# lightas/CVPR2020_MANet

Measured on AMD Instinct MI355X. Metric: propagated frames/sec at 480p, 5-frame memory, higher is better.
Workload: dtype f32; 1 GPU; BASELINE configs[1]: grid 120x214, C=100, 5-frame fully-labelled bank (M=128400), 2 ids, f32 arithmetic on f32-stored iid embeddings; step = frame prepare + global match + fused normalise/min-merge + local match d=12; bank sorted/packed once per clip, timed; frames_per_gpu=633, clip_frames=633, bank_exchange=none (1 GPU)

## Files before the change

### cvpr2020_manet_amd/csrc/global_match.hip

```cpp
#include "manet_common.h"
#include <type_traits>
#include "local_geom.h"

namespace {

constexpr int QT = 256;
constexpr int QB = 32;
constexpr int BT = 64;
constexpr int META_INTS = 256;
constexpr int META_T = 0;
constexpr int META_SEG = 1;
constexpr int META_CNT = 130;
constexpr int META_KMAX = 200;
constexpr int META_NAN = 66;
int refine_sub(long T_max) { return T_max <= 2500 ? 8 : 16; }
constexpr int REFINE_XCHG_MASK = 3;
constexpr int REFINE_CAP = 128;
constexpr int REFINE_LDS_LIST = 2048;
constexpr int REFINE_DENSE_CAP = 1024;
constexpr unsigned REFINE_DENSE_BIT = 0x80000000u;
constexpr int REFINE_DENSE_MIN = 64;
constexpr int REFINE_DENSE_LANES = 16;
constexpr int REFINE_RZ = 4;
constexpr int ONE_ROUND_OK = 1 << 29;
// ... 670 lines not shown
    return (u & 0x80000000u) ? ~u : (u | 0x80000000u);
}
__device__ __forceinline__ float float_of(unsigned k)
{
    unsigned u = (k & 0x80000000u) ? (k & 0x7fffffffu) : ~k;
    return __uint_as_float(u);
}

__device__ __forceinline__ float min3p(float m, float a, float b)
{
    return __builtin_elementwise_minimum(__builtin_elementwise_minimum(m, a), b);
}

constexpr int FILTER_TAIL_CUTS = 4;
__device__ __forceinline__ bool split_of_block(int b, int nQT, int S, int T, int block_map, int &qt, int &s, int &t0,
                                               int &t1)
{
    const int bm = block_map & 0xff, small_S = (block_map >> 8) & BLOCK_MAP_SMALL_S_MASK;
    bool one_round = T < S && small_S > 0;
    if (!one_round && (block_map & ONE_ROUND_OK) && small_S > 0 && small_S < S) {
        const float rounds = (float)nQT * (float)S / 512.0f;
        const float whole = floorf(rounds), frac = rounds - whole;
        const float last = frac <= 0.0f ? 0.0f : (frac <= 0.5f ? 0.5f : 1.0f);
        const float cost_host = (whole + last) * ((float)T / (float)S + 0.6f);
        const float cost_one = ceilf((float)T / (float)small_S) + 0.6f;
        one_round = cost_one < 0.97f * cost_host;
    }
    if (one_round) {
        const int S2 = small_S < T ? small_S : T;
        qt = b % nQT;
        s = b / nQT;
        if (s >= S2) return false;
        t0 = (int)((long)s * T / S2);
        t1 = (int)((long)(s + 1) * T / S2);
        return t0 < t1;
    }
    if (bm == 0 || bm == 3) {
        const int xcd = b & 7;
        const int idx = b >> 3;
        qt = idx % nQT;
        s = xcd + 8 * (idx / nQT);
        if (bm == 3 && (S & 7) == 0) s = xcd * (S >> 3) + idx / nQT;
    } else if (bm >= 4 && bm <= 7 && (S & 7) == 0) {
        const int PB = bm - 2, S8 = S >> 3;
        const int xcd = b & 7, idx = b >> 3;
        const int g = idx / (nQT * PB), r = idx - g * (nQT * PB);
        const int pbg = (S8 - g * PB) < PB ? (S8 - g * PB) : PB;
        if (pbg <= 0) return false;
        qt = r / pbg;
        s = xcd + 8 * (g * PB + (r - qt * pbg));
        if (qt >= nQT) return false;
    } else if (bm == 1) {
        qt = b % nQT;
        s = b / nQT;
    } else {
        s = b % S;
        qt = b / S;
    }
    t0 = (int)((long)s * T / S);
    t1 = (int)((long)(s + 1) * T / S);
    return t0 < t1;
}

__device__ __forceinline__ bool tapered_split_of_block(int b, int nQT, int S, int T, int &qt, int &s, int &t0, int &t1)
{
    const int xcd = b & 7, idx = b >> 3, S8 = S >> 3;
    const int full = nQT * (S8 - 1);
    int cut = 0, cuts = 1;
    if (idx < full) {
        qt = idx % nQT;
        s = xcd * S8 + idx / nQT;
    } else {
        const int r = idx - full;
        cut = r / nQT;
        cuts = FILTER_TAIL_CUTS;
        if (cut >= FILTER_TAIL_CUTS) return false;
        qt = r - cut * nQT;
        s = xcd * S8 + S8 - 1;
    }
    const int a = (int)((long)s * T / S), e = (int)((long)(s + 1) * T / S);
    t0 = a + (int)((long)cut * (e - a) / cuts);
    t1 = a + (int)((long)(cut + 1) * (e - a) / cuts);
    return t0 < t1;
}


template <int K>
__device__ __forceinline__ void topk_insert(float (&m)[K], float d)
{
#pragma unroll
    for (int j = 0; j < K; ++j) {
        float lo = fminf(m[j], d);
        d = fmaxf(m[j], d);
        m[j] = lo;
    }
}

template <int KS, int KNN, bool ARG = false, bool NTH = false>
__global__ __launch_bounds__(256, ((KS == 64 && (KNN > 1 || ARG)) || NTH) ? 1 : 2) void global_match_f32_kernel(const char *__restrict__ qpack,
                                                                  const char *__restrict__ bpack,
                                                                  const int *__restrict__ meta,
                                                                  int n_ids, int nQT, int S,
                                                                  long N_pad,
                                                                  unsigned *__restrict__ keys,
                                                                  float *__restrict__ topk, int block_map)
{
    static_assert(!ARG || KNN == 1, "arg-min tracking is the k = 1 path");
    static_assert(!NTH || ARG, "the bounded form is a variant of the arg-min form");
    unsigned long long *keys64 = (unsigned long long *)topk;
    const unsigned long long *bound64 = (const unsigned long long *)keys;
    constexpr int NG = (KS + 3) / 4;
    constexpr size_t TILE_BYTES = bank_tile_bytes(NG);
    constexpr size_t QBLK_BYTES = query_block_bytes(NG);
    extern __shared__ __attribute__((aligned(16))) char smem[];

    const int tid = threadIdx.x;
    const int lane = tid & 63;
    const int wave = __builtin_amdgcn_readfirstlane(tid >> 6);
    const int l31 = lane & 31;
    const int h = lane >> 5;

    int qt, s, t0, t1;
    const int T = meta[META_T];
    if (!split_of_block(blockIdx.x, nQT, S, T, block_map, qt, s, t0, t1)) return;

    constexpr int NV = (int)(TILE_BYTES / 16);
    constexpr int NLD = (NV + 255) / 256;
    u32x4 R[NLD];
#define MANET_GLOAD(R_, t_)                                                                \
    {                                                                                      \
        const u32x4 *g_ = (const u32x4 *)(bpack + (size_t)(t_) * TILE_BYTES);              \
        _Pragma("unroll") for (int i_ = 0; i_ < NLD; ++i_)                                 \
        {                                                                                  \
            const int idx_ = i_ * NTHR + tid;                                              \
            R_[i_] = g_[idx_ < NV ? idx_ : NV - 1];   \
        }                                                                                  \
    }
#define MANET_LSTORE(R_, slot_)                                                            \
    {                                                                                      \
        u32x4 *l_ = (u32x4 *)(smem + (size_t)(slot_) * TILE_BYTES);                        \
        _Pragma("unroll") for (int i_ = 0; i_ < NLD; ++i_)                                 \
            if (i_ * NTHR + tid < NV) l_[i_ * NTHR + tid] = R_[i_];                        \
    }
    constexpr int NTHR = 256;
    MANET_GLOAD(R, t0);

    f32x4 q0[NG], q1[NG];
    float xs0, xs1;
    {
        const char *qb0 = qpack + (size_t)(qt * (QT / QB) + wave * 2) * QBLK_BYTES;
        const char *qb1 = qb0 + QBLK_BYTES;
#pragma unroll
        for (int g = 0; g < NG; ++g) {
            q0[g] = *(const f32x4 *)(qb0 + ((size_t)(g * 2 + h) * QB + l31) * 16);
            q1[g] = *(const f32x4 *)(qb1 + ((size_t)(g * 2 + h) * QB + l31) * 16);
        }
        xs0 = *(const float *)(qb0 + (size_t)NG * 2 * QB * 16 + l31 * 4);
        xs1 = *(const float *)(qb1 + (size_t)NG * 2 * QB * 16 + l31 * 4);
    }
    const long qbase = (long)qt * QT + wave * 64 + l31;

    int o = 0;
    while (meta[META_SEG + o + 1] <= t0) ++o;
    int seg_end = meta[META_SEG + o + 1];
    float m0[KNN], m1[KNN];
    int a0 = -1, a1 = -1;
    unsigned long long B0 = ~0ull, B1 = ~0ull, lo0 = 0, lo1 = 0;
    auto reset = [&]() {
#pragma unroll
        for (int j = 0; j < KNN; ++j) m0[j] = m1[j] = (KNN == 1) ? MANET_WRONG_LABEL_PADDING_DISTANCE : INFINITY;
        a0 = a1 = -1;
        B0 = B1 = ~0ull;
    };
    auto load_bounds = [&](int obj) {
        if (NTH) {
            lo0 = bound64[(size_t)obj * N_pad + qbase];
            lo1 = bound64[(size_t)obj * N_pad + qbase + 32];
        }
    };
    reset();
    load_bounds(o);

    auto flush = [&](int obj) {
        if (ARG) {
            unsigned long long k0 = ((unsigned long long)key_of(m0[0]) << 32) | (unsigned)(a0 < 0 ? -1 : a0 + 4 * h);
            unsigned long long k1 = ((unsigned long long)key_of(m1[0]) << 32) | (unsigned)(a1 < 0 ? -1 : a1 + 4 * h);
            if (NTH) {
                k0 = B0;
                k1 = B1;
            }
            const unsigned long long o0 = __shfl_xor(k0, 32), o1 = __shfl_xor(k1, 32);
            k0 = k0 < o0 ? k0 : o0;
            k1 = k1 < o1 ? k1 : o1;
            if (h == 0) {
                atomicMin(keys64 + (size_t)obj * N_pad + qbase, k0);
                atomicMin(keys64 + (size_t)obj * N_pad + qbase + 32, k1);
            }
        } else if (KNN == 1) {
            float a = min3p(m0[0], m0[0], __shfl_xor(m0[0], 32));
            float c = min3p(m1[0], m1[0], __shfl_xor(m1[0], 32));
            if (h == 0) {
                atomicMin(keys + (size_t)obj * N_pad + qbase, key_of(a));
                atomicMin(keys + (size_t)obj * N_pad + qbase + 32, key_of(c));
            }
        } else {
            float o0[KNN], o1[KNN];
#pragma unroll
            for (int j = 0; j < KNN; ++j) {
                o0[j] = __shfl_xor(m0[j], 32);
                o1[j] = __shfl_xor(m1[j], 32);
            }
#pragma unroll
            for (int j = 0; j < KNN; ++j) {
                topk_insert<KNN>(m0, o0[j]);
                topk_insert<KNN>(m1, o1[j]);
            }
            if (h == 0) {
                float *p0 = topk + (((size_t)s * n_ids + obj) * N_pad + qbase) * KNN;
                float *p1 = p0 + (size_t)32 * KNN;
#pragma unroll
                for (int j = 0; j < KNN; ++j) {
                    p0[j] = m0[j];
                    p1[j] = m1[j];
                }
            }
        }
    };

    MANET_LSTORE(R, 0);
    if (t0 + 1 < t1) MANET_GLOAD(R, t0 + 1);
    for (int t = t0; t < t1; ++t) {
        const int buf = (t - t0) & 1;
        __syncthreads();
        if (t + 1 < t1) {
            MANET_LSTORE(R, buf ^ 1);
            if (t + 2 < t1) MANET_GLOAD(R, t + 2);
        }
        if (t >= seg_end) {
            flush(o);
            reset();
            do { ++o; seg_end = meta[META_SEG + o + 1]; } while (t >= seg_end);
            load_bounds(o);
        }
        const char *tb = smem + (size_t)buf * TILE_BYTES;
        const f32x4 *A = (const f32x4 *)tb;
        f32x16 c00 = {0}, c01 = {0}, c10 = {0}, c11 = {0};
#pragma unroll
        for (int g = 0; g < NG; ++g) {
            f32x4 a0 = A[(g * 2 + h) * BT + l31];
            f32x4 a1 = A[(g * 2 + h) * BT + 32 + l31];
#pragma unroll
            for (int j = 0; j < 4; ++j) {
                if (g * 4 + j < KS) {
                    c00 = __builtin_amdgcn_mfma_f32_32x32x2f32(a0[j], q0[g][j], c00, 0, 0, 0);
                    c01 = __builtin_amdgcn_mfma_f32_32x32x2f32(a0[j], q1[g][j], c01, 0, 0, 0);
                    c10 = __builtin_amdgcn_mfma_f32_32x32x2f32(a1[j], q0[g][j], c10, 0, 0, 0);
                    c11 = __builtin_amdgcn_mfma_f32_32x32x2f32(a1[j], q1[g][j], c11, 0, 0, 0);
                }
            }
        }
        const float *ysl = (const float *)(tb + (size_t)NG * 2 * BT * 16);
#pragma unroll
        for (int tq = 0; tq < 4; ++tq) {
            f32x4 y0 = *(const f32x4 *)(ysl + 8 * tq + 4 * h);
            f32x4 y1 = *(const f32x4 *)(ysl + 32 + 8 * tq + 4 * h);
#pragma unroll
            for (int i = 0; i < 4; ++i) {
                const int r = 4 * tq + i;
                const float d00 = fmaf(-2.0f, c00[r], xs0 + y0[i]);
                const float d01 = fmaf(-2.0f, c01[r], xs1 + y0[i]);
                const float d10 = fmaf(-2.0f, c10[r], xs0 + y1[i]);
                const float d11 = fmaf(-2.0f, c11[r], xs1 + y1[i]);
                if (NTH) {
                    const unsigned slot = (unsigned)(t * BT + (r & 3) + 8 * (r >> 2) + 4 * h);
                    const unsigned long long k00 = ((unsigned long long)key_of(d00) << 32) | slot;
                    const unsigned long long k10 = ((unsigned long long)key_of(d10) << 32) | (slot + 32u);
                    const unsigned long long k01 = ((unsigned long long)key_of(d01) << 32) | slot;
                    const unsigned long long k11 = ((unsigned long long)key_of(d11) << 32) | (slot + 32u);
                    if (k00 > lo0 && k00 < B0) B0 = k00;
                    if (k10 > lo0 && k10 < B0) B0 = k10;
                    if (k01 > lo1 && k01 < B1) B1 = k01;
                    if (k11 > lo1 && k11 < B1) B1 = k11;
                } else if (ARG) {
                    const int slot = t * BT + (r & 3) + 8 * (r >> 2);
                    if (d00 < m0[0]) { m0[0] = d00; a0 = slot; }
                    if (d10 < m0[0]) { m0[0] = d10; a0 = slot + 32; }
                    if (d01 < m1[0]) { m1[0] = d01; a1 = slot; }
                    if (d11 < m1[0]) { m1[0] = d11; a1 = slot + 32; }
                } else if (KNN == 1) {
                    m0[0] = min3p(m0[0], d00, d10);
                    m1[0] = min3p(m1[0], d01, d11);
                } else {
                    topk_insert<KNN>(m0, d00);
                    topk_insert<KNN>(m0, d10);
                    topk_insert<KNN>(m1, d01);
                    topk_insert<KNN>(m1, d11);
                }
            }
        }
    }
    flush(o);
}

template <int KS, bool RESCUE = false>
__global__ __launch_bounds__(256, 2) void global_match_f32_pipe_kernel(const char *__restrict__ qpack,
                                                                       const char *__restrict__ bpack,
                                                                       const int *__restrict__ meta, int n_ids,
                                                                       int nQT, int S, long N_pad,
                                                                       unsigned *__restrict__ keys, int block_map,
                                                                       const unsigned *__restrict__ bcnt = nullptr,
                                                                       long bucket_cap = 0)
{
    constexpr int NG = (KS + 3) / 4;
    constexpr size_t TILE_BYTES = bank_tile_bytes(NG);
    constexpr size_t QBLK_BYTES = query_block_bytes(NG);
    constexpr int PIECES = (int)(TILE_BYTES / 1024);
    constexpr int NW = 4;
    extern __shared__ __attribute__((aligned(16))) char smem[];

    const int tid = threadIdx.x;
    const int lane = tid & 63;
    const int wave = __builtin_amdgcn_readfirstlane(tid >> 6);
    const int l31 = lane & 31;
    const int h = lane >> 5;

    int qt, s, t0, t1;
    const int T = meta[META_T];
    if (RESCUE && (block_map & RESCUE_LISTED)) {
        const unsigned *rs = bcnt + 2 * (N_pad >> 5);
        const int nr = (int)rs[0];
        if (nr <= 0) return;
        int Sd = (block_map >> 8) & BLOCK_MAP_RESCUE_MASK;
        if (Sd > 0) {
            const int most_grid = (int)gridDim.x / nr;
            Sd = Sd > most_grid ? most_grid : Sd;
            Sd = Sd < 1 ? 1 : Sd;
        } else {
            const int most_grid = (int)gridDim.x / nr, most_t = T / 8 > 1 ? T / 8 : 1;
            const int most = most_grid < most_t ? most_grid : most_t;
            long best = -1;
            for (int r = 1; r <= 4; ++r) {
                int c = (512 * r) / nr;
                c = c < 1 ? 1 : (c > most ? most : c);
                const long rounds = ((long)nr * c + 511) / 512;
                const long cost = rounds * ((long)(T + c - 1) / c + 6);
                if (best < 0 || cost < best) { best = cost; Sd = c; }
            }
        }
        if ((int)blockIdx.x >= nr * Sd) return;
        s = (int)blockIdx.x / nr;
        qt = (int)rs[1 + ((int)blockIdx.x - s * nr)];
        t0 = (int)((long)s * T / Sd);
        t1 = (int)((long)(s + 1) * T / Sd);
        if (t0 >= t1) return;
    } else {
        if (!split_of_block(blockIdx.x, nQT, S, T, block_map, qt, s, t0, t1)) return;
        if (RESCUE) {
            bool need = false;
            for (int i = 0; i < QT / QB; ++i) {
                const unsigned raw = bcnt[(long)qt * (QT / QB) + i];
                need = need || (raw >> 31) || (long)raw > bucket_cap;
            }
            if (!need) return;
        }
    }

    const unsigned smem_base = __builtin_amdgcn_readfirstlane((unsigned)(size_t)smem);
    auto stage_dma = [&](int t, int slot) __attribute__((always_inline)) {
        const char *g = bpack + (size_t)t * TILE_BYTES + (size_t)lane * 16;
        const unsigned l = smem_base + (unsigned)slot * (unsigned)TILE_BYTES;
#pragma unroll
        for (int i = 0; i < (PIECES + NW - 1) / NW; ++i) {
            const int pc = wave + i * NW;
            if (pc < PIECES) lds_dma16(g + (size_t)pc * 1024, l + (unsigned)pc * 1024u);
        }
    };
    stage_dma(t0, 0);

    f32x4 q0[NG], q1[NG];
    float xs0, xs1;
    {
        const char *qb0 = qpack + (size_t)(qt * (QT / QB) + wave * 2) * QBLK_BYTES;
        const char *qb1 = qb0 + QBLK_BYTES;
#pragma unroll
        for (int g = 0; g < NG; ++g) {
            q0[g] = *(const f32x4 *)(qb0 + ((size_t)(g * 2 + h) * QB + l31) * 16);
            q1[g] = *(const f32x4 *)(qb1 + ((size_t)(g * 2 + h) * QB + l31) * 16);
        }
        xs0 = *(const float *)(qb0 + (size_t)NG * 2 * QB * 16 + l31 * 4);
        xs1 = *(const float *)(qb1 + (size_t)NG * 2 * QB * 16 + l31 * 4);
    }
    const long qbase = (long)qt * QT + wave * 64 + l31;
#pragma unroll
    for (int g = 0; g < NG; ++g) asm volatile("" : "+v"(q0[g]), "+v"(q1[g]));
    asm volatile("" : "+v"(xs0), "+v"(xs1));

    int o = 0;
    while (meta[META_SEG + o + 1] <= t0) ++o;
    int seg_end = meta[META_SEG + o + 1];
    float m0a, m0b, m1a, m1b;
    m0a = m0b = m1a = m1b = MANET_WRONG_LABEL_PADDING_DISTANCE;
    auto flush = [&](int obj) {
        const float v0 = min3p(m0a, m0b, m0b), v1 = min3p(m1a, m1b, m1b);
        const float a = min3p(v0, v0, __shfl_xor(v0, 32));
        const float c = min3p(v1, v1, __shfl_xor(v1, 32));
        if (h == 0) {
            atomicMin(keys + (size_t)obj * N_pad + qbase, key_of(a));
            atomicMin(keys + (size_t)obj * N_pad + qbase + 32, key_of(c));
        }
    };

    f32x16 c00 = {0}, c01 = {0}, c10 = {0}, c11 = {0};
    float yp[16];
#pragma unroll
    for (int r = 0; r < 16; ++r) yp[r] = MANET_WRONG_LABEL_PADDING_DISTANCE;
#define MANET_REDUCE(ca_, cb_, y_, r_)                                                             \
    {                                                                                              \
        const float da_ = fmaf(-2.0f, ca_[r_], xs0 + (y_));                                        \
        const float db_ = fmaf(-2.0f, cb_[r_], xs1 + (y_));                                        \
        if ((r_) & 1) {                                                                            \
            m0b = min3p(m0b, da_, da_);                                                            \
            m1b = min3p(m1b, db_, db_);                                                            \
        } else {                                                                                   \
            m0a = min3p(m0a, da_, da_);                                                            \
            m1a = min3p(m1a, db_, db_);                                                            \
        }                                                                                          \
    }
    auto settle = [&]() __attribute__((always_inline)) {
#pragma unroll
        for (int r = 0; r < 16; ++r) MANET_REDUCE(c10, c11, yp[r], r);
#pragma unroll
        for (int r = 0; r < 16; ++r) yp[r] = MANET_WRONG_LABEL_PADDING_DISTANCE;
        c10 = f32x16{0};
        c11 = f32x16{0};
    };

    for (int t = t0; t < t1; ++t) {
        const int buf = (t - t0) & 1;
        asm volatile("s_waitcnt vmcnt(0)" ::: "memory");
        __builtin_amdgcn_s_barrier();
        asm volatile("" ::: "memory");
        if (t + 1 < t1) stage_dma(t + 1, buf ^ 1);
        if (t >= seg_end) {
            settle();
            flush(o);
            m0a = m0b = m1a = m1b = MANET_WRONG_LABEL_PADDING_DISTANCE;
            do { ++o; seg_end = meta[META_SEG + o + 1]; } while (t >= seg_end);
        }
        const char *tb = smem + (size_t)buf * TILE_BYTES;
        const f32x4 *A = (const f32x4 *)tb;
        const float *ysl = (const float *)(tb + (size_t)NG * 2 * BT * 16);
        c00 = f32x16{0};
        c01 = f32x16{0};
#pragma unroll
        for (int g = 0; g < NG; ++g) {
            const f32x4 a0 = A[(g * 2 + h) * BT + l31];
#pragma unroll
            for (int j = 0; j < 4; ++j) {
                if (g * 4 + j < KS) {
                    c00 = __builtin_amdgcn_mfma_f32_32x32x2f32(a0[j], q0[g][j], c00, 0, 0, 0);
                    c01 = __builtin_amdgcn_mfma_f32_32x32x2f32(a0[j], q1[g][j], c01, 0, 0, 0);
                }
            }
#pragma unroll
            for (int r = (g * 16) / NG; r < ((g + 1) * 16) / NG; ++r) MANET_REDUCE(c10, c11, yp[r], r);
        }
#pragma unroll
        for (int tq = 0; tq < 4; ++tq) {
            const f32x4 y1 = *(const f32x4 *)(ysl + 32 + 8 * tq + 4 * h);
#pragma unroll
            for (int i = 0; i < 4; ++i) yp[4 * tq + i] = y1[i];
        }
        c10 = f32x16{0};
        c11 = f32x16{0};
        f32x4 y0v[4];
#pragma unroll
        for (int tq = 0; tq < 4; ++tq) y0v[tq] = *(const f32x4 *)(ysl + 8 * tq + 4 * h);
#pragma unroll
        for (int g = 0; g < NG; ++g) {
            const f32x4 a1 = A[(g * 2 + h) * BT + 32 + l31];
#pragma unroll
            for (int j = 0; j < 4; ++j) {
                if (g * 4 + j < KS) {
                    c10 = __builtin_amdgcn_mfma_f32_32x32x2f32(a1[j], q0[g][j], c10, 0, 0, 0);
                    c11 = __builtin_amdgcn_mfma_f32_32x32x2f32(a1[j], q1[g][j], c11, 0, 0, 0);
                }
            }
#pragma unroll
            for (int r = (g * 16) / NG; r < ((g + 1) * 16) / NG; ++r) MANET_REDUCE(c00, c01, y0v[r >> 2][r & 3], r);
        }
    }
    settle();
#undef MANET_REDUCE
    flush(o);
}

template <int KSB>
__global__ __launch_bounds__(512, 1) void global_match_bf16x3_kernel(const char *__restrict__ qpack,
                                                                     const char *__restrict__ bpack,
                                                                     const int *__restrict__ meta, int n_ids,
                                                                     int nQT, int S, long N_pad,
                                                                     unsigned *__restrict__ keys, int block_map)
{
    typedef __bf16 bf16x8_t __attribute__((ext_vector_type(8)));
    constexpr int NW = 8;
    constexpr int UNITS = 4 * KSB;
    constexpr int LO = 2 * KSB;
    constexpr size_t TILE_BYTES = bank_tile_bytes_u(UNITS, false);
    constexpr size_t QBLK_BYTES = query_block_bytes_u(UNITS, false);
    constexpr int QTB = NW * 64;
    static_assert(TILE_BYTES == (size_t)UNITS * 1024, "a bf16 tile is a whole number of 1 KiB DMA pieces");
    extern __shared__ __attribute__((aligned(16))) char smem[];

    const int tid = threadIdx.x;
    const int lane = tid & 63;
    const int wave = __builtin_amdgcn_readfirstlane(tid >> 6);
    const int l31 = lane & 31;
    const int h = lane >> 5;

    int qt, s, t0, t1;
    const int T = meta[META_T];
    if (!split_of_block(blockIdx.x, nQT, S, T, block_map, qt, s, t0, t1)) return;

    const unsigned smem_base = __builtin_amdgcn_readfirstlane((unsigned)(size_t)smem);
    auto stage_dma = [&](int t, int slot) __attribute__((always_inline)) {
        const int np = ((t1 - t) < 1 ? (t1 - t) : 1) * UNITS;
        const char *g = bpack + (size_t)t * TILE_BYTES + (size_t)lane * 16;
        const unsigned l = smem_base + (unsigned)slot * (unsigned)TILE_BYTES;
#pragma unroll
        for (int i = 0; i < (UNITS + NW - 1) / NW; ++i) {
            const int pc = wave + i * NW;
            if (pc < np) lds_dma16(g + (size_t)pc * 1024, l + (unsigned)pc * 1024u);
        }
    };
    stage_dma(t0, 0);

    u32x4 q0[KSB], q1[KSB], q0l[KSB], q1l[KSB];
    {
        const char *qb0 = qpack + (size_t)(qt * (QTB / QB) + wave * 2) * QBLK_BYTES;
        const char *qb1 = qb0 + QBLK_BYTES;
#pragma unroll
        for (int k = 0; k < KSB; ++k) {
            q0[k] = *(const u32x4 *)(qb0 + ((size_t)(k * 2 + h) * QB + l31) * 16);
            q1[k] = *(const u32x4 *)(qb1 + ((size_t)(k * 2 + h) * QB + l31) * 16);
            q0l[k] = *(const u32x4 *)(qb0 + ((size_t)(LO + k * 2 + h) * QB + l31) * 16);
            q1l[k] = *(const u32x4 *)(qb1 + ((size_t)(LO + k * 2 + h) * QB + l31) * 16);
        }
    }
    const long qbase = (long)qt * QTB + wave * 64 + l31;
#pragma unroll
    for (int k = 0; k < KSB; ++k) {
        asm volatile("" : "+v"(q0[k]), "+v"(q1[k]));
        asm volatile("" : "+v"(q0l[k]), "+v"(q1l[k]));
    }

    int o = 0;
    while (meta[META_SEG + o + 1] <= t0) ++o;
    int seg_end = meta[META_SEG + o + 1];
    float m0a, m0b, m1a, m1b;
    m0a = m0b = m1a = m1b = MANET_WRONG_LABEL_PADDING_DISTANCE;
    auto flush = [&](int obj) {
        float a = min3p(m0a, m0b, __shfl_xor(min3p(m0a, m0b, m0b), 32));
        float c = min3p(m1a, m1b, __shfl_xor(min3p(m1a, m1b, m1b), 32));
        if (h == 0) {
            atomicMin(keys + (size_t)obj * N_pad + qbase, key_of(a));
            atomicMin(keys + (size_t)obj * N_pad + qbase + 32, key_of(c));
        }
    };
#define MANET_BF(x) __builtin_bit_cast(bf16x8_t, x)
#define MANET_MFMA(a_, b_, c_) c_ = __builtin_amdgcn_mfma_f32_32x32x16_bf16(MANET_BF(a_), MANET_BF(b_), c_, 0, 0, 0)
    auto tile = [&](const char *tb) __attribute__((always_inline)) {
        const u32x4 *A = (const u32x4 *)tb;
        f32x16 c00 = {0}, c01 = {0}, c10 = {0}, c11 = {0};
#pragma unroll
        for (int k = 0; k < KSB; ++k) {
            u32x4 a0 = A[(k * 2 + h) * BT + l31];
            u32x4 a1 = A[(k * 2 + h) * BT + 32 + l31];
            u32x4 a0l = A[(LO + k * 2 + h) * BT + l31];
            u32x4 a1l = A[(LO + k * 2 + h) * BT + 32 + l31];
            MANET_MFMA(a0, q0[k], c00);
            MANET_MFMA(a1, q0[k], c10);
            MANET_MFMA(a0, q1[k], c01);
            MANET_MFMA(a1, q1[k], c11);
            MANET_MFMA(a0, q0l[k], c00);
            MANET_MFMA(a1, q0l[k], c10);
            MANET_MFMA(a0, q1l[k], c01);
            MANET_MFMA(a1, q1l[k], c11);
            MANET_MFMA(a0l, q0[k], c00);
            MANET_MFMA(a1l, q0[k], c10);
            MANET_MFMA(a0l, q1[k], c01);
            MANET_MFMA(a1l, q1[k], c11);
        }
#pragma unroll
        for (int r = 0; r < 16; r += 2) {
            m0a = min3p(m0a, c00[r], c10[r]);
            m0b = min3p(m0b, c00[r + 1], c10[r + 1]);
            m1a = min3p(m1a, c01[r], c11[r]);
            m1b = min3p(m1b, c01[r + 1], c11[r + 1]);
        }
    };
    auto next_object = [&](int t) __attribute__((always_inline)) {
        if (t >= seg_end) {
            flush(o);
            m0a = m0b = m1a = m1b = MANET_WRONG_LABEL_PADDING_DISTANCE;
            do { ++o; seg_end = meta[META_SEG + o + 1]; } while (t >= seg_end);
        }
    };
    int buf = 0;
    for (int t = t0; t < t1; ++t, buf ^= 1) {
        asm volatile("s_waitcnt vmcnt(0)" ::: "memory");
        __builtin_amdgcn_s_barrier();
        asm volatile("" ::: "memory");
        if (t + 1 < t1) stage_dma(t + 1, buf ^ 1);
        next_object(t);
        tile(smem + (size_t)buf * TILE_BYTES);
    }
#undef MANET_MFMA
#undef MANET_BF
    flush(o);
}

template <int KSB>
__global__ __launch_bounds__(512, 1) __attribute__((amdgpu_waves_per_eu(2, 2)))
void global_match_bf16_pipe_kernel(const char *__restrict__ qpack, const char *__restrict__ bpack,
                                   const int *__restrict__ meta, int n_ids, int nQT, int S, long N_pad,
                                   unsigned *__restrict__ keys, int block_map)
{
    typedef __bf16 bf16x8_t __attribute__((ext_vector_type(8)));
    constexpr int NW = 8, TPS = 2;
    constexpr int UNITS = 2 * KSB;
    constexpr size_t TILE_BYTES = bank_tile_bytes_u(UNITS, false);
    constexpr size_t QBLK_BYTES = query_block_bytes_u(UNITS, false);
    constexpr size_t STEP_BYTES = TILE_BYTES * TPS;
    constexpr int QTB = NW * 64;
    constexpr int NBUF = 2;
    extern __shared__ __attribute__((aligned(16))) char smem[];

    const int tid = threadIdx.x;
    const int lane = tid & 63;
    const int wave = __builtin_amdgcn_readfirstlane(tid >> 6);
    const int l31 = lane & 31;
    const int h = lane >> 5;

    int qt, s, t0, t1;
    const int T = meta[META_T];
    if (!split_of_block(blockIdx.x, nQT, S, T, block_map, qt, s, t0, t1)) return;

    constexpr int PIECES = UNITS * TPS;
    const unsigned smem_base = __builtin_amdgcn_readfirstlane((unsigned)(size_t)smem);
    auto stage_dma = [&](int t, int slot) __attribute__((always_inline)) {
        const int np = ((t1 - t) < TPS ? (t1 - t) : TPS) * UNITS;
        const char *g = bpack + (size_t)t * TILE_BYTES + (size_t)lane * 16;
        const unsigned l = smem_base + (unsigned)slot * (unsigned)STEP_BYTES;
#pragma unroll
        for (int i = 0; i < (PIECES + NW - 1) / NW; ++i) {
            const int pc = wave + i * NW;
            if (pc < np) lds_dma16(g + (size_t)pc * 1024, l + (unsigned)pc * 1024u);
        }
    };
    stage_dma(t0, 0);
    if (t0 + TPS < t1) stage_dma(t0 + TPS, 1);

    u32x4 q0[KSB], q1[KSB];
    {
        const char *qb0 = qpack + (size_t)(qt * (QTB / QB) + wave * 2) * QBLK_BYTES;
        const char *qb1 = qb0 + QBLK_BYTES;
#pragma unroll
        for (int k = 0; k < KSB; ++k) {
            q0[k] = *(const u32x4 *)(qb0 + ((size_t)(k * 2 + h) * QB + l31) * 16);
            q1[k] = *(const u32x4 *)(qb1 + ((size_t)(k * 2 + h) * QB + l31) * 16);
        }
    }
    const long qbase = (long)qt * QTB + wave * 64 + l31;
#pragma unroll
    for (int k = 0; k < KSB; ++k) asm volatile("" : "+v"(q0[k]), "+v"(q1[k]));

    int o = 0;
    while (meta[META_SEG + o + 1] <= t0) ++o;
    int seg_end = meta[META_SEG + o + 1];
    float m0a, m0b, m1a, m1b;
    m0a = m0b = m1a = m1b = MANET_WRONG_LABEL_PADDING_DISTANCE;
    auto flush = [&](int obj) {
        float a = min3p(m0a, m0b, __shfl_xor(min3p(m0a, m0b, m0b), 32));
        float c = min3p(m1a, m1b, __shfl_xor(min3p(m1a, m1b, m1b), 32));
        if (h == 0) {
            atomicMin(keys + (size_t)obj * N_pad + qbase, key_of(a));
            atomicMin(keys + (size_t)obj * N_pad + qbase + 32, key_of(c));
        }
    };
    auto next_object = [&](int t) __attribute__((always_inline)) {
        if (t >= seg_end) {
            flush(o);
            m0a = m0b = m1a = m1b = MANET_WRONG_LABEL_PADDING_DISTANCE;
            do { ++o; seg_end = meta[META_SEG + o + 1]; } while (t >= seg_end);
        }
    };
    const unsigned frag_off = (unsigned)((h * BT + l31) * 16);
    u32x4 F0[KSB], F1[KSB];
#define MANET_BF(x) __builtin_bit_cast(bf16x8_t, x)
#define MANET_MFMA(a_, b_, c_) c_ = __builtin_amdgcn_mfma_f32_32x32x16_bf16(MANET_BF(a_), MANET_BF(b_), c_, 0, 0, 0)
#define MANET_LOADF(k_, tile_base_)                                                                \
    {                                                                                              \
        const char *f_ = (tile_base_) + frag_off + (size_t)(k_) * (2 * BT * 16);                   \
        F0[k_] = *(const u32x4 *)f_;                                                               \
        F1[k_] = *(const u32x4 *)(f_ + 32 * 16);                                                   \
    }
#define MANET_TILE(next_base_)                                                                     \
    {                                                                                              \
        f32x16 c00 = {0}, c01 = {0}, c10 = {0}, c11 = {0};                                         \
        _Pragma("unroll") for (int k = 0; k < KSB; ++k)                                            \
        {                                                                                          \
            MANET_MFMA(F0[k], q0[k], c00);                                                         \
            MANET_MFMA(F1[k], q0[k], c10);                                                         \
            MANET_MFMA(F0[k], q1[k], c01);                                                         \
            MANET_MFMA(F1[k], q1[k], c11);                                                         \
            MANET_LOADF(k, next_base_);                                                            \
            __builtin_amdgcn_sched_group_barrier(0x008, 4, 0);                        \
            __builtin_amdgcn_sched_group_barrier(0x100, 2, 0);  \
        }                                                                                          \
        _Pragma("unroll") for (int r = 0; r < 16; r += 2)                                          \
        {                                                                                          \
            m0a = min3p(m0a, c00[r], c10[r]);                                                      \
            m0b = min3p(m0b, c00[r + 1], c10[r + 1]);                                              \
            m1a = min3p(m1a, c01[r], c11[r]);                                                      \
            m1b = min3p(m1b, c01[r + 1], c11[r + 1]);                                              \
        }                                                                                          \
    }

    asm volatile("s_waitcnt vmcnt(0)" ::: "memory");
    __builtin_amdgcn_s_barrier();
    asm volatile("" ::: "memory");
#pragma unroll
    for (int k = 0; k < KSB; ++k) MANET_LOADF(k, smem);

    int buf = 0;
    for (int t = t0; t < t1; t += TPS, buf ^= 1) {
        const char *cur = smem + (size_t)buf * STEP_BYTES;
        const char *nxt = smem + (size_t)(buf ^ 1) * STEP_BYTES;
        next_object(t);
        MANET_TILE(cur + TILE_BYTES);
        asm volatile("s_waitcnt vmcnt(0)" ::: "memory");
        asm volatile("s_waitcnt lgkmcnt(0)" ::: "memory");
        __builtin_amdgcn_s_barrier();
        asm volatile("" ::: "memory");
        if (t + NBUF * TPS < t1) stage_dma(t + NBUF * TPS, buf);
        if (t + 1 < t1) {
            next_object(t + 1);
            MANET_TILE(nxt);
        }
    }
#undef MANET_TILE
#undef MANET_LOADF
#undef MANET_MFMA
#undef MANET_BF
    flush(o);
}

template <int KSB, bool FILTER = false>
__global__ __launch_bounds__(256, 2) void global_match_bf16_wide_kernel(const char *__restrict__ qpack,
                                                                        const char *__restrict__ bpack,
                                                                        const int *__restrict__ meta, int n_ids,
                                                                        int nQT, int S, long N_pad,
                                                                        unsigned *__restrict__ keys, int block_map,
                                                                        unsigned *__restrict__ thr,
                                                                        const float *__restrict__ slack,
                                                                        unsigned long long *__restrict__ stats,
                                                                        uint2 *__restrict__ list, long bucket_cap,
                                                                        unsigned *__restrict__ bcnt)
{
    typedef __bf16 bf16x8_t __attribute__((ext_vector_type(8)));
    constexpr int NW = 4, TPS = 2, NQB = 4;
    constexpr int UNITS = 2 * KSB;
    constexpr size_t TILE_BYTES = bank_tile_bytes_u(UNITS, false);
    constexpr size_t QBLK_BYTES = query_block_bytes_u(UNITS, false);
    constexpr size_t STEP_BYTES = TILE_BYTES * TPS;
    constexpr int QTB = QT_BF16;
    static_assert(NW * NQB * QB == QTB, "4 waves x 4 blocks x 32 queries");
    extern __shared__ __attribute__((aligned(16))) char smem[];

    const int tid = threadIdx.x;
    const int lane = tid & 63;
    const int wave = __builtin_amdgcn_readfirstlane(tid >> 6);
    const int l31 = lane & 31;
    const int h = lane >> 5;

    int qt, s, t0, t1;
    const int T = meta[META_T];
    if (FILTER && (block_map & 0xff) == 8) {
        if (!tapered_split_of_block(blockIdx.x, nQT, S, T, qt, s, t0, t1)) return;
    } else if (!split_of_block(blockIdx.x, nQT, S, T, block_map, qt, s, t0, t1))
        return;

    constexpr int PIECES = UNITS * TPS;
// ... 1545 lines not shown
```

Measured before the change: 211.4 frames/s.

## Software-pipeline LDS fragment loads and interleave MFMA with reductions in f32 pipe kernel

Restructures the f32 global-match inner loop into compile-time unrolled steps that prefetch the next bank fragment from LDS into a double-buffered register while the current MFMAs run. Explicit sched_group_barrier hints interleave the min-reduction VALU work between MFMAs, and the next tile's DMA is issued after the first step instead of before. The goal is to hide LDS latency and keep the matrix units busy. In exchange it adds more register pressure and rigid scheduling constraints, and it needs an extra lgkmcnt wait at the barrier.

```diff
diff --git a/cvpr2020_manet_amd/csrc/global_match.hip b/cvpr2020_manet_amd/csrc/global_match.hip
--- a/cvpr2020_manet_amd/csrc/global_match.hip
+++ b/cvpr2020_manet_amd/csrc/global_match.hip
@@ -996,6 +996,14 @@
     flush(o);
 }
 
+template <int I0, int I1, class Fn>
+__device__ __forceinline__ void each_step(Fn &f)
+{
+    if constexpr (I0 < I1) {
+        f(std::integral_constant<int, I0>{});
+        each_step<I0 + 1, I1>(f);
+    }
+}
 template <int KS, bool RESCUE = false>
 __global__ __launch_bounds__(256, 2) void global_match_f32_pipe_kernel(const char *__restrict__ qpack,
                                                                        const char *__restrict__ bpack,
@@ -1064,8 +1072,12 @@
         const char *g = bpack + (size_t)t * TILE_BYTES + (size_t)lane * 16;
         const unsigned l = smem_base + (unsigned)slot * (unsigned)TILE_BYTES;
 #pragma unroll
-        for (int i = 0; i < (PIECES + NW - 1) / NW; ++i) {
+        for (int i = 0; i < PIECES / NW; ++i) {
             const int pc = wave + i * NW;
+            lds_dma16(g + (size_t)pc * 1024, l + (unsigned)pc * 1024u);
+        }
+        if (PIECES % NW) {
+            const int pc = wave + (PIECES / NW) * NW;
             if (pc < PIECES) lds_dma16(g + (size_t)pc * 1024, l + (unsigned)pc * 1024u);
         }
     };
@@ -1129,60 +1141,77 @@
         c11 = f32x16{0};
     };
 
+    const unsigned frag_off = (unsigned)((h * BT + l31) * 16);
+    f32x4 F[2], y0v[4];
+    const char *tb;
+    auto step = [&](auto st_) __attribute__((always_inline)) {
+        constexpr int ST = decltype(st_)::value, PH = ST / NG, G = ST % NG;
+        constexpr int NM = 2 * (KS - 4 * G < 4 ? KS - 4 * G : 4);
+        constexpr int R0 = (G * 16) / NG, R1 = ((G + 1) * 16) / NG;
+        constexpr int YQ = PH == 0 ? G - (NG - 4) : G;
+        constexpr bool YREAD = YQ >= 0 && YQ < 4;
+        constexpr int PER = (6 * (R1 - R0) + NM - 2) / (NM - 1);
+        const float *ysl = (const float *)(tb + (size_t)NG * 2 * BT * 16);
+        if (ST + 1 < 2 * NG) {
+            constexpr int PH1 = (ST + 1) / NG, G1 = (ST + 1) % NG;
+            F[(ST + 1) & 1] = *(const f32x4 *)(tb + frag_off + (size_t)(G1 * 2 * BT + 32 * PH1) * 16);
+        }
+        if (YREAD) {
+            if (PH == 0) {
+                y0v[YQ] = *(const f32x4 *)(ysl + 8 * YQ + 4 * h);
+            } else {
+                const f32x4 y1 = *(const f32x4 *)(ysl + 32 + 8 * YQ + 4 * h);
+#pragma unroll
+                for (int i = 0; i < 4; ++i) yp[4 * YQ + i] = y1[i];
+            }
+        }
+        const f32x4 a = F[ST & 1];
+        if (NM < 8) asm volatile("" ::"v"(a));
+#pragma unroll
+        for (int j = 0; j < NM / 2; ++j) {
+            if (PH == 0) {
+                c00 = __builtin_amdgcn_mfma_f32_32x32x2f32(a[j], q0[G][j], G + j ? c00 : f32x16{0}, 0, 0, 0);
+                c01 = __builtin_amdgcn_mfma_f32_32x32x2f32(a[j], q1[G][j], G + j ? c01 : f32x16{0}, 0, 0, 0);
+            } else {
+                c10 = __builtin_amdgcn_mfma_f32_32x32x2f32(a[j], q0[G][j], G + j ? c10 : f32x16{0}, 0, 0, 0);
+                c11 = __builtin_amdgcn_mfma_f32_32x32x2f32(a[j], q1[G][j], G + j ? c11 : f32x16{0}, 0, 0, 0);
+            }
+        }
+#pragma unroll
+        for (int r = R0; r < R1; ++r) {
+            if (PH == 0) {
+                MANET_REDUCE(c10, c11, yp[r], r);
+            } else {
+                MANET_REDUCE(c00, c01, y0v[r >> 2][r & 3], r);
+            }
+        }
+        __builtin_amdgcn_sched_group_barrier(0x008, 1, 0);
+        __builtin_amdgcn_sched_group_barrier(0x100, (ST + 1 < 2 * NG) + YREAD, 0);
+#pragma unroll
+        for (int j = 1; j < NM; ++j) {
+            __builtin_amdgcn_sched_group_barrier(0x002, PER, 0);
+            __builtin_amdgcn_sched_group_barrier(0x008, 1, 0);
+        }
+        __builtin_amdgcn_sched_barrier(0);
+    };
+
     for (int t = t0; t < t1; ++t) {
         const int buf = (t - t0) & 1;
-        asm volatile("s_waitcnt vmcnt(0)" ::: "memory");
+        asm volatile("s_waitcnt vmcnt(0) lgkmcnt(0)" ::: "memory");
         __builtin_amdgcn_s_barrier();
         asm volatile("" ::: "memory");
-        if (t + 1 < t1) stage_dma(t + 1, buf ^ 1);
         if (t >= seg_end) {
             settle();
             flush(o);
             m0a = m0b = m1a = m1b = MANET_WRONG_LABEL_PADDING_DISTANCE;
             do { ++o; seg_end = meta[META_SEG + o + 1]; } while (t >= seg_end);
         }
-        const char *tb = smem + (size_t)buf * TILE_BYTES;
-        const f32x4 *A = (const f32x4 *)tb;
-        const float *ysl = (const float *)(tb + (size_t)NG * 2 * BT * 16);
-        c00 = f32x16{0};
-        c01 = f32x16{0};
-#pragma unroll
-        for (int g = 0; g < NG; ++g) {
-            const f32x4 a0 = A[(g * 2 + h) * BT + l31];
-#pragma unroll
-            for (int j = 0; j < 4; ++j) {
-                if (g * 4 + j < KS) {
-                    c00 = __builtin_amdgcn_mfma_f32_32x32x2f32(a0[j], q0[g][j], c00, 0, 0, 0);
-                    c01 = __builtin_amdgcn_mfma_f32_32x32x2f32(a0[j], q1[g][j], c01, 0, 0, 0);
-                }
-            }
-#pragma unroll
-            for (int r = (g * 16) / NG; r < ((g + 1) * 16) / NG; ++r) MANET_REDUCE(c10, c11, yp[r], r);
-        }
-#pragma unroll
-        for (int tq = 0; tq < 4; ++tq) {
-            const f32x4 y1 = *(const f32x4 *)(ysl + 32 + 8 * tq + 4 * h);
-#pragma unroll
-            for (int i = 0; i < 4; ++i) yp[4 * tq + i] = y1[i];
-        }
-        c10 = f32x16{0};
-        c11 = f32x16{0};
-        f32x4 y0v[4];
-#pragma unroll
-        for (int tq = 0; tq < 4; ++tq) y0v[tq] = *(const f32x4 *)(ysl + 8 * tq + 4 * h);
-#pragma unroll
-        for (int g = 0; g < NG; ++g) {
-            const f32x4 a1 = A[(g * 2 + h) * BT + 32 + l31];
-#pragma unroll
-            for (int j = 0; j < 4; ++j) {
-                if (g * 4 + j < KS) {
-                    c10 = __builtin_amdgcn_mfma_f32_32x32x2f32(a1[j], q0[g][j], c10, 0, 0, 0);
-                    c11 = __builtin_amdgcn_mfma_f32_32x32x2f32(a1[j], q1[g][j], c11, 0, 0, 0);
-                }
-            }
-#pragma unroll
-            for (int r = (g * 16) / NG; r < ((g + 1) * 16) / NG; ++r) MANET_REDUCE(c00, c01, y0v[r >> 2][r & 3], r);
-        }
+        tb = smem + (size_t)buf * TILE_BYTES;
+        F[0] = *(const f32x4 *)(tb + frag_off);
+        __builtin_amdgcn_sched_barrier(0);
+        step(std::integral_constant<int, 0>{});
+        if (t + 1 < t1) stage_dma(t + 1, buf ^ 1);
+        each_step<1, 2 * NG>(step);
     }
     settle();
 #undef MANET_REDUCE
```

After: 207.2 frames/s. 0.98x the previous value.
